# skeskinen/bert.cpp

Measured on AMD Instinct MI355X. Metric: sentences/sec (seq_len=128), higher is better.
Workload: dtype f16; 1 GPU; all-MiniLM-L6-v2 f16, batch=256 seq_len=128; per_gpu_batch=256, global_batch=256, seq_len=128, weights=f16, parallelism=dp1 (replicated weights, sharded sentences)

## Files before the change

bert.cpp_amd/csrc/device.h:

```cpp
#pragma once
#include "kernels.h"

#include <cstdio>
#include <type_traits>
#include <utility>

namespace bert_hip {

typedef _Float16 f16x2 __attribute__((ext_vector_type(2)));
typedef _Float16 f16x4 __attribute__((ext_vector_type(4)));
typedef _Float16 f16x8 __attribute__((ext_vector_type(8)));
typedef float f32x2 __attribute__((ext_vector_type(2)));
typedef float f32x4 __attribute__((ext_vector_type(4)));
typedef float f32x8 __attribute__((ext_vector_type(8)));
typedef float f32x16 __attribute__((ext_vector_type(16)));
typedef uint32_t u32x4 __attribute__((ext_vector_type(4)));
typedef uint32_t u32x16 __attribute__((ext_vector_type(16)));
typedef int32_t i32x4 __attribute__((ext_vector_type(4)));
typedef int32_t i32x16 __attribute__((ext_vector_type(16)));

template <int... I, class F>
__device__ __forceinline__ void static_for_impl(std::integer_sequence<int, I...>, F &&f) {
    (f(std::integral_constant<int, I>{}), ...);
}
// ... 52 lines not shown
}
template <bool MEMORY, int OFF, class V = f16x8>
__device__ __forceinline__ V lds_read_b128(unsigned addr) {
    static_assert(sizeof(V) == 16, "ds_read_b128 reads 16 bytes");
    static_assert(OFF >= 0 && OFF < 65536, "ds offset field is 16 bits");
    V v;
    if constexpr (MEMORY) asm volatile("ds_read_b128 %0, %1 offset:%2" : "=v"(v) : "v"(addr), "n"(OFF) : "memory");
    else asm volatile("ds_read_b128 %0, %1 offset:%2" : "=v"(v) : "v"(addr), "n"(OFF));
    return v;
}
template <class V>
__device__ __forceinline__ void landed(V &v) { asm volatile("" : "+v"(v)); }
template <int VM>
__device__ __forceinline__ void dma_barrier() {
    asm volatile("s_waitcnt vmcnt(%0) lgkmcnt(0)\n\ts_barrier" : : "n"(VM) : "memory");
}

__device__ __forceinline__ int off64(int row, int chunk) { return row * 128 + ((chunk ^ ((row >> 1) & 7)) << 4); }

__device__ __forceinline__ float rounded_f32(float v) {
    asm("" : "+v"(v));
    return v;
}

__device__ __forceinline__ void xor32_pair(float &a, float &b) {
    asm("s_nop 1\n\tv_permlane32_swap_b32 %0, %1\n\ts_nop 1" : "+v"(a), "+v"(b));
}
__device__ __forceinline__ f16x8 result_to_operand_fragment(const f16x8 &v) {
    const u32x4 d = __builtin_bit_cast(u32x4, v);
    uint32_t d0 = d[0], d1 = d[1], d2 = d[2], d3 = d[3];
    asm("s_nop 1\n\tv_permlane32_swap_b32 %0, %2\n\tv_permlane32_swap_b32 %1, %3\n\ts_nop 1" : "+v"(d0), "+v"(d1), "+v"(d2), "+v"(d3));
    return __builtin_bit_cast(f16x8, u32x4{d0, d1, d2, d3});
}
__device__ __forceinline__ float xor32_sum(float v) { float a = v, b = v; xor32_pair(a, b); return a + b; }
__device__ __forceinline__ float xor32_max(float v) { float a = v, b = v; xor32_pair(a, b); return __builtin_fmaxf(a, b); }
__device__ __forceinline__ float wave_sum_f32(float v) {
    v = xor32_sum(v);
    v += __builtin_bit_cast(float, __builtin_amdgcn_ds_swizzle(__builtin_bit_cast(int, v), (16 << 10) | 0x1F));
    v += __builtin_bit_cast(float, __builtin_amdgcn_ds_swizzle(__builtin_bit_cast(int, v), (8 << 10) | 0x1F));
    v += __builtin_bit_cast(float, __builtin_amdgcn_ds_swizzle(__builtin_bit_cast(int, v), (4 << 10) | 0x1F));
    v += __builtin_bit_cast(float, __builtin_amdgcn_mov_dpp(__builtin_bit_cast(int, v), 0x4E, 0xF, 0xF, true));
    v += __builtin_bit_cast(float, __builtin_amdgcn_mov_dpp(__builtin_bit_cast(int, v), 0xB1, 0xF, 0xF, true));
    return v;
}

#ifndef BERT_HIP_EXP16
#define BERT_HIP_EXP16 0
#endif
#if BERT_HIP_EXP16
typedef u32x4 sm_arg_t;
typedef u32x4 sm_exp_t;
__device__ __forceinline__ sm_arg_t softmax_args4(float s0, float s1, float s2, float s3, float s4, float s5, float s6, float s7, float sc, float m) {
    uint32_t a0, a1, a2, a3;
    asm("v_fma_mixlo_f16 %0, %4, %12, -%13\n\t"
        "v_fma_mixlo_f16 %1, %6, %12, -%13\n\t"
        "v_fma_mixlo_f16 %2, %8, %12, -%13\n\t"
        "v_fma_mixlo_f16 %3, %10, %12, -%13\n\t"
        "v_fma_mixhi_f16 %0, %5, %12, -%13\n\t"
        "v_fma_mixhi_f16 %1, %7, %12, -%13\n\t"
        "v_fma_mixhi_f16 %2, %9, %12, -%13\n\t"
        "v_fma_mixhi_f16 %3, %11, %12, -%13"
        : "=&v"(a0), "=&v"(a1), "=&v"(a2), "=&v"(a3)
        : "v"(s0), "v"(s1), "v"(s2), "v"(s3), "v"(s4), "v"(s5), "v"(s6), "v"(s7), "s"(sc), "v"(m));
    return u32x4{a0, a1, a2, a3};
}
__device__ __forceinline__ sm_exp_t softmax_exp4(sm_arg_t a) {
// ... 214 lines not shown
```

bert.cpp_amd/csrc/engine.hip:

```cpp
#include "engine.h"

#include <algorithm>
#include <cstdio>
#include <cstdlib>
#include <chrono>
#include <cstring>
#include <system_error>
#include <thread>

namespace bert_hip {

#define HIP_OK(expr, errvar, ret)                                                                       \
    do {                                                                                                \
        hipError_t e__ = (expr);                                                                        \
        if (e__ != hipSuccess) {                                                                        \
            errvar = std::string(#expr) + ": " + hipGetErrorString(e__);                                \
            return ret;                                                                                 \
        }                                                                                               \
    } while (0)

DevBuf::~DevBuf() {
    if (p) (void)hipFree(p);
}
bool DevBuf::alloc(size_t n, std::string &err) {
// ... 349 lines not shown
    HIP_OK(hipDeviceSynchronize(), err, -1);
    int st = 0;
    HIP_OK(hipMemcpy(&st, status_.p, sizeof(int), hipMemcpyDeviceToHost), err, -1);
    if (st) HIP_OK(hipMemset(status_.p, 0, sizeof(int)), err, -1);
    return st;
}

void Engine::set_option(const std::string &key, const std::string &value) {
#ifndef BERT_HIP_TEST_ROUTES
    if ((key == "gemm" || key == "attn") && value == "naive") {
        fprintf(stderr, "bert_hip_set_option: %s=naive is a test cross-check (libbert_test.so), not a route of libbert.so; ignored\n", key.c_str());
        return;
    }
#endif
    if (key == "gemm") {
        bool have = true;
        for (auto *L : layers_)
            for (GemmWeightStore *w : {&L->qkv, &L->o, &L->ffi, &L->ffo}) have = have && w->w.naive16 != nullptr;
        if (value == "naive" && !have)
            fprintf(stderr, "bert_hip_set_option: gemm=naive needs BERT_HIP_KERNELS=naive at load time (the f16 row-major images were not built); ignored\n");
        else gemm_naive_ = value == "naive";
    } else if (key == "attn") attn_naive_ = value == "naive";
    else if (key == "qkv2") qkv2_ = value != "0";
    else if (key == "gemm256") gemm256_ = value != "0";
    else if (key == "ln_fold" && value != "0" && !fold_images_)
        fprintf(stderr, "bert_hip_set_option: ln_fold=1 needs BERT_HIP_LN_FOLD=1 at load time (the folded images were not built); ignored\n");
    else if (key == "ln_fold") ln_fold_ = value != "0";
    else if (key == "tail") tail_ = value != "0";
    else if (key == "latency") latency_ = value != "0";
    else if (key == "stage_kernel") stage_kernel_ = value != "0";
    else if (key == "window_slots") set_window_slots(atoi(value.c_str()));
    else if (key == "latency_tokens") { const int v = atoi(value.c_str()); if (v >= 32) latency_tokens_ = v; }
    else if (key == "one_launch") one_launch_ = value == "0" ? 0 : value == "2" ? 2 : 1;
    else if (key == "f32") f32_exact_ = value != "f16";
    else if (key == "chunk_tokens") { const int v = atoi(value.c_str()); if (v > 0) chunk_tokens_ = v; }
    else if (key == "profile_replay") {
        const size_t c = value.rfind(':');
        replay_name_ = c == std::string::npos ? value : value.substr(0, c);
        replay_k_ = c == std::string::npos ? 10 : std::max(1, atoi(value.c_str() + c + 1));
    }
}

bool Engine::ensure_workspace(int t_pad, int n_sentences, std::string &err) {
    const size_t H = hp_.n_embd, I = hp_.n_intermediate, tp = (size_t)t_pad;
    const size_t es = f32_file_ ? 4 : 2;
    return x_.ensure(tp * H * es, err) && qkv_.ensure(tp * 3 * H * es, err) && ctx_.ensure(tp * H * es, err) &&
           y_.ensure(tp * H * es, err) && ff_.ensure(tp * I * es, err) && v32_.ensure((size_t)std::max(128, std::min(t_pad, (latency_tokens_ + 255) / 256 * 256)) * H * 4, err) &&
           d_out_.ensure((size_t)n_sentences * H * 4, err) &&
           windows_.ensure((size_t)n_sentences * sizeof(int2), err) &&
           (!(H > 384 && H % 256 == 0) || (ln_stats1_.ensure(tp * (2 * H / 256) * 8, err) && ln_stats2_.ensure(tp * (2 * H / 256) * 8, err) &&
                                           ln_rows1_.ensure(tp * 16, err) && ln_rows2_.ensure(tp * 16, err)));
}

template <class F>
void Engine::timed(const char *name, double flops, hipStream_t s, F &&f) {
    if (!profiling_) { f(); return; }
    auto get = [&]() {
        hipEvent_t ev;
        if (!ev_pool_.empty()) { ev = ev_pool_.back(); ev_pool_.pop_back(); }
        else (void)hipEventCreate(&ev);
        return ev;
    };
    if (!replay_name_.empty()) {
        f();
        if (replay_done_ || replay_name_ != name) return;
        replay_done_ = true;
// ... 453 lines not shown
```

bert.cpp_amd/csrc/layer_tail.hip:

```cpp
#include "device.h"

namespace bert_hip {

namespace {

constexpr int LT_TILE = 16384;
#ifndef LT_ABLATE
#define LT_ABLATE 0
#endif
#ifndef LT_UPRIO
#define LT_UPRIO 1
#endif
#ifndef LT_GELU_BATCH
#define LT_GELU_BATCH 0
#endif
#ifndef LT_DMA_SPLIT
#define LT_DMA_SPLIT 1
#endif
#ifndef LT_DPRIO
#define LT_DPRIO 0
#endif

#ifdef BERT_HIP_TIMELINE
static __device__ unsigned long long g_tl_tail[256 * 512];
// ... 25 lines not shown
    asm volatile("s_waitcnt lgkmcnt(%4)" : "+v"(f[0]), "+v"(f[1]), "+v"(f[2]), "+v"(f[3]) : "n"(N) : "memory");
}
template <int N>
__device__ __forceinline__ void wait_lgkm() {
    asm volatile("s_waitcnt lgkmcnt(%0)" : : "n"(N) : "memory");
}
template <int VM>
__device__ __forceinline__ void close_interval(f16x8 (&f)[4]) {
    asm volatile("s_waitcnt vmcnt(%4) lgkmcnt(0)\n\ts_barrier" : "+v"(f[0]), "+v"(f[1]), "+v"(f[2]), "+v"(f[3]) : "n"(VM) : "memory");
}
template <int OFF>
__device__ __forceinline__ f16x8 frag_read(unsigned addr) {
    if (LT_ABLATE & 4) { f16x8 z = (f16x8)(_Float16)0.f; asm volatile("" : "+v"(z) : "v"(addr)); return z; }
    return lds_read_b128<true, OFF>(addr);
}

__device__ __forceinline__ void dma_m0(unsigned lds) {
    if (LT_ABLATE & 1) return;
    asm volatile("s_mov_b32 m0, %0" : : "s"(lds) : "memory");
}
template <int PIECE>
__device__ __forceinline__ void dma_piece(const char *gbase, unsigned voff) {
    if (LT_ABLATE & 1) return;
    asm volatile("global_load_lds_dwordx4 %0, %1 offset:%2" : : "v"(voff), "s"(gbase - PIECE * 1024), "n"(PIECE * 1024) : "memory");
}

__device__ __forceinline__ f32x16 mfma16(const f16x8 &a, const f16x8 &b, const f32x16 &c) {
    if (LT_ABLATE & 8) { f32x16 r = c; asm volatile("" : "+v"(r[0]) : "v"(a), "v"(b)); return r; }
    return __builtin_amdgcn_mfma_f32_32x32x16_f16(a, b, c, 0, 0, 0);
}

}

template <int NT, int WT, bool RAGGED, bool HANDOVER>
__device__ __forceinline__ void layer_tail_body(const TailArgs &a, char *smem, const int tok0, const int rows, const int tid,
                                                [[maybe_unused]] f16x8 (&xnext)[8 * NT]) {
    static_assert(!(HANDOVER && RAGGED), "a ragged window's rows are packed: its lanes are not the window phase's slots");
    constexpr bool Q4 = WT != GW_F16;
    constexpr int VMQ = Q4 ? 63 : 0;
    constexpr int H = 128 * NT, NBH = 2 * NT, NB = 4 * NT, NQ = 8 * NT, NYH = 4 * NT;
    constexpr int P = NT * NT;
    constexpr int NG = NT;
    constexpr int LAGT = NT + NG;
    const int I = a.I, NC = I / 64;
    const int lane = tid & 63;
    const int wave = __builtin_amdgcn_readfirstlane(tid >> 6);
    const int t = wave & 3, role = wave >> 2;
    const int l31 = lane & 31, hi = lane >> 5;
    const int tok_w = tok0 + t * 32;
    const int row_l = RAGGED ? tok0 + min(t * 32 + l31, rows - 1) : tok_w + l31;

    char *ringU = smem;
    char *ringD = smem + 3 * LT_TILE;
    char *G = smem + 6 * LT_TILE;
    float *ST = (float *)(G + 32768);
    float *cbo = ST + 8 * 64;
    float *cg1 = cbo + H, *cbe1 = cg1 + H, *cb2 = cbe1 + H, *cg2 = cb2 + H, *cbe2 = cg2 + H, *cb1 = cbe2 + H;

    {
        constexpr int NPB = 4;
        const float *const src[6] = {a.bo, a.g1, a.be1, a.b2, a.g2, a.be2};
        float pv[6];
        f32x4 bq[NPB];
#pragma unroll
        for (int k = 0; k < 6; ++k) pv[k] = tid < H ? src[k][tid] : 0.f;
#pragma unroll
        for (int k = 0; k < NPB; ++k) {
            const int i4 = (k * 512 + tid) * 4;
            bq[k] = i4 < I ? *(const f32x4 *)(a.b1 + i4) : f32x4{0.f, 0.f, 0.f, 0.f};
        }
        if (tid < H) {
#pragma unroll
            for (int k = 0; k < 6; ++k) cbo[k * H + tid] = pv[k];
        }
#pragma unroll
        for (int k = 0; k < NPB; ++k) {
            const int i4 = (k * 512 + tid) * 4;
            if (i4 < I + 128) *(f32x4 *)(cb1 + i4) = bq[k];
        }
    }
    f32x16 accp[NBH];
    f16x4 xv[NBH][4];
    {
        const half_t *xr = a.x + (size_t)row_l * H + role * 64 + 4 * hi;
#pragma unroll
        for (int b = 0; b < NBH; ++b)
#pragma unroll
            for (int gq = 0; gq < 4; ++gq) xv[b][gq] = *(const f16x4 *)(xr + (b >> 1) * 128 + (b & 1) * 32 + 8 * gq);
    }
    f16x8 bf[NQ];
    {
        const half_t *cw = a.ctx + (size_t)row_l * H + 8 * hi;
#pragma unroll
        for (int q = 0; q < NQ; ++q) bf[q] = *(const f16x8 *)(cw + 16 * q);
    }

    auto rows_offset = [&](int pitch) __attribute__((always_inline)) {
        int ln = lane;
        asm volatile("" : "+v"(ln));
        const int ch0 = (ln & 7) ^ (ln >> 4), row = t * 32 + (ln >> 3);
        return (unsigned)(row * pitch * 2 + ch0 * 16);
    };
    const half_t *const wo = a.wo, *const w1p = a.w1p, *const w2p = a.w2p;
    auto dma128 = [&](const half_t *base, unsigned oe, int row_bytes, unsigned tile) __attribute__((always_inline)) {
        const char *b = (const char *)base;
        dma_m0(tile + (unsigned)(t * 4096));
        dma_piece<0>(b, oe);
        dma_piece<1>(b + (size_t)8 * row_bytes, oe ^ 64u);
        dma_piece<2>(b + (size_t)16 * row_bytes, oe);
        dma_piece<3>(b + (size_t)24 * row_bytes, oe ^ 64u);
    };
    const unsigned ldsU = lds_addr(ringU), ldsD = lds_addr(ringD);
    const unsigned offH = rows_offset(H);
    auto up_offset = [&]() __attribute__((always_inline)) {
        int ln = lane;
        asm volatile("" : "+v"(ln));
        return (unsigned)((t * 16 + (ln >> 4)) * H * 2 + (((ln & 15) ^ (ln >> 4)) * 16));
    };
    auto dma_up_f16 = [&](int c, int j, unsigned offU, unsigned tile) __attribute__((always_inline)) {
        const char *b = (const char *)(w1p + (size_t)c * 64 * H + j * 128);
        dma_m0(tile + (unsigned)(t * 4096));
        dma_piece<0>(b, offU);
        dma_piece<1>(b + (size_t)4 * H * 2, offU ^ 64u);
        dma_piece<2>(b + (size_t)8 * H * 2, offU ^ 128u);
// ... 43 lines not shown
    const unsigned aUp = lds_addr(ringU) + (unsigned)(l31 * 256 + ((hi ^ (l31 & 15)) << 4));

    int slot = 0;
    [[maybe_unused]] int tl = 1;
    [[maybe_unused]] const bool tlU = tid == 0, tlD = tid == 256;
    LT_STAMP(tlU, 0);
    auto pre_close = [&]() __attribute__((always_inline)) { LT_STAMP_FINE(tlU, 128 + tl); LT_STAMP_FINE(tlD, 256 + tl); };
    auto next_slot = [&]() __attribute__((always_inline)) { slot = slot == 2 ? 0 : slot + 1; LT_STAMP(tlU, tl); ++tl; };
    auto slot_plus2 = [&]() __attribute__((always_inline)) { return slot == 0 ? 2 : slot - 1; };
    [[maybe_unused]] auto slot_plus1 = [&]() __attribute__((always_inline)) { return slot == 2 ? 0 : slot + 1; };
    using PLAIN = std::false_type; using PERMUTED = std::true_type;

    auto proj_request = [&](int p, int s) __attribute__((always_inline)) {
        const int n3 = p / NT, q = p % NT;
        if (role == 0) dma_proj(n3, 2 * q, ldsU + s * LT_TILE);
        else dma_proj(n3, 2 * q + 1, ldsD + s * LT_TILE);
    };
    proj_request(0, 0);
    q4_expand_rows(PLAIN{}, role ? ringD : ringU);
    proj_request(1, 1);
    LT_STAMP(tlU, 384);
    asm volatile("s_waitcnt vmcnt(0) lgkmcnt(0)\n\ts_barrier" ::: "memory");
    LT_STAMP(tlU, 385);
#pragma unroll
    for (int b = 0; b < NBH; ++b)
#pragma unroll
        for (int gq = 0; gq < 4; ++gq) {
            const f32x4 bv = *(const f32x4 *)(cbo + (b >> 1) * 128 + role * 64 + (b & 1) * 32 + 8 * gq + 4 * hi);
#pragma unroll
            for (int e = 0; e < 4; ++e) accp[b][4 * gq + e] = (float)xv[b][gq][e] + bv[e];
        }
#pragma unroll
    for (int b = 0; b < NBH; ++b) asm volatile("" : "+v"(accp[b]));
    __builtin_amdgcn_s_waitcnt(0xc07f);
    static_for<P>([&](auto p_tag) __attribute__((always_inline)) {
        constexpr int p = decltype(p_tag)::value, n3 = p / NT, q = p % NT, p2 = p + 2;
        const unsigned bA = aR + (unsigned)(slot * LT_TILE + role * 8192), bB = bA + 3 * LT_TILE;
        f16x8 Fa[4], Fb[4];
        auto rd = [&](unsigned base, int g2, f16x8 (&F)[4]) __attribute__((always_inline)) {
            const unsigned a0 = base ^ (unsigned)((2 * g2) << 5), a1 = base ^ (unsigned)((2 * g2 + 1) << 5);
            F[0] = frag_read<0>(a0); F[1] = frag_read<4096>(a0);
            F[2] = frag_read<0>(a1); F[3] = frag_read<4096>(a1);
        };
        auto mm = [&](f16x8 (&F)[4], int ks) __attribute__((always_inline)) {
            accp[n3 * 2 + 0] = mfma16(F[0], bf[ks], accp[n3 * 2 + 0]);
            accp[n3 * 2 + 1] = mfma16(F[1], bf[ks], accp[n3 * 2 + 1]);
            accp[n3 * 2 + 0] = mfma16(F[2], bf[ks + 1], accp[n3 * 2 + 0]);
            accp[n3 * 2 + 1] = mfma16(F[3], bf[ks + 1], accp[n3 * 2 + 1]);
        };
        auto q4_turn = [&]() __attribute__((always_inline)) {
            if constexpr (p + 1 < P) q4_expand_rows(PLAIN{}, (role ? ringD : ringU) + slot_plus1() * LT_TILE);
            else if (role == 1) q4_expand_up(ringU + slot_plus1() * LT_TILE);
            const int s2 = slot_plus2();
            if constexpr (p2 < P) proj_request(p2, s2);
            else if (role == 1) dma_up(0, p2 - P, up_offset(), ldsU + s2 * LT_TILE);
        };
        constexpr int QW = Q4 && p + 1 < P ? 4 : 0;
        if constexpr (LT_ABLATE & 64) {
            if constexpr (Q4) q4_turn();
            else {
                const int s2 = slot_plus2();
                if constexpr (p2 < P) proj_request(p2, s2);
                else if (role == 1) dma_up(0, p2 - P, up_offset(), ldsU + s2 * LT_TILE);
            }
            pre_close();
            if (p2 < P || role == 1) dma_barrier<Q4 ? 63 : 4>(); else dma_barrier<VMQ>();
            next_slot();
            return;
        }
        rd(bA, 0, Fa);
        rd(bA, 1, Fb);
        if constexpr (!Q4) {
            const int s2 = slot_plus2();
            if constexpr (p2 < P) proj_request(p2, s2);
            else if (role == 1) dma_up(0, p2 - P, up_offset(), ldsU + s2 * LT_TILE);
        }
        wait_frags<4>(Fa);
        mm(Fa, 8 * q + 0);
        __builtin_amdgcn_sched_barrier(0);
        rd(bB, 0, Fa);
        wait_frags<4>(Fb);
        mm(Fb, 8 * q + 2);
        __builtin_amdgcn_sched_barrier(0);
        rd(bB, 1, Fb);
        if constexpr (Q4) { q4_turn(); __builtin_amdgcn_sched_barrier(0); }
        wait_frags<4 + QW>(Fa);
        mm(Fa, 8 * q + 4);
        __builtin_amdgcn_sched_barrier(0);
        wait_frags<0>(Fb);
        mm(Fb, 8 * q + 6);
        __builtin_amdgcn_sched_barrier(0);
        pre_close();
        if (p2 < P || role == 1) dma_barrier<Q4 ? 63 : 4>(); else dma_barrier<VMQ>();
        next_slot();
    });

    if (role == 1) q4_expand_up(ringU + slot_plus1() * LT_TILE);
    LT_STAMP(tlU, 386); LT_STAMP(tlD, 396);
    float ln_rstd, ln_nmr;
    {
        float s1 = 0.f, s2 = 0.f;
#pragma unroll
        for (int b = 0; b < ((LT_ABLATE & 32) ? 0 : NBH); ++b)
#pragma unroll
            for (int r = 0; r < 16; ++r) { s1 += accp[b][r]; s2 = __builtin_fmaf(accp[b][r], accp[b][r], s2); }
        s1 += __shfl_xor(s1, 32);
        s2 += __shfl_xor(s2, 32);
        if (hi == 0) *(f32x2 *)(ST + wave * 64 + l31 * 2) = f32x2{s1, s2};
        LT_STAMP(tlU, 387); LT_STAMP(tlD, 397);
        asm volatile("s_waitcnt lgkmcnt(0)\n\ts_barrier" ::: "memory");
        LT_STAMP(tlU, 388);
        const f32x2 o = *(const f32x2 *)(ST + (wave ^ 4) * 64 + l31 * 2);
        s1 += o[0]; s2 += o[1];
        layernorm_scale(s1, s2, 1.0f / H, ln_rstd, ln_nmr);
    }
    auto normalise_block = [&](auto b_tag, f16x8 &y0, f16x8 &y1) __attribute__((always_inline)) {
        constexpr int b = decltype(b_tag)::value;
        const int f0 = (b >> 1) * 128 + role * 64 + (b & 1) * 32 + 4 * hi;
        if constexpr (LT_ABLATE & 32) {
#pragma unroll
            for (int e = 0; e < 8; ++e) { y0[e] = (_Float16)accp[b][e]; y1[e] = (_Float16)accp[b][8 + e]; }
            return;
// ... 466 lines not shown
```

bert.cpp_amd/csrc/model_kernel.hip:

```cpp
#define BERT_HIP_PHASES_ONLY
#include "qkv_attention2.hip"
#include "layer_tail.hip"
#undef BERT_HIP_PHASES_ONLY
#include "pool_normalize.h"

namespace bert_hip {

#ifdef BERT_HIP_MODEL_TIMELINE
static __device__ unsigned long long g_tl_model[1024 * 32];
#define MK_STAMP(i) do { const int mk_i = (i); if (threadIdx.x == 0 && mk_i < 32) g_tl_model[(blockIdx.x & 1023) * 32 + mk_i] = __builtin_amdgcn_s_memrealtime(); } while (0)
#else
#define MK_STAMP(i) do { } while (0)
#endif

namespace {

constexpr int MODEL_MAX_LAYERS = 12;

struct ModelLayerArgs {
    const half_t *wqkv, *wo, *w1p, *w2p;
    const float *bqkv, *bo, *g1, *be1, *b1, *b2, *g2, *be2;
};
struct ModelArgs {
    half_t *x, *ctx;
    const int32_t *cu;
    const int2 *groups;
    const int *n_groups;
    int n_layer, n_head, n_sent, I, slot_mask;
    float *pooled;
    int *status;
    int max_len;
    ModelLayerArgs layer[MODEL_MAX_LAYERS];
};

}

template <int NT, bool RAGGED>
__global__ __launch_bounds__(512, 2) void model_kernel(ModelArgs m) {
    extern __shared__ __attribute__((aligned(16))) char smem[];
    const int window = (int)blockIdx.x;
    int tok0 = window * 128, rows = 128, first = window, count = 1;
    if constexpr (RAGGED) {
        if (m.groups) {
            if (m.n_groups && window >= *m.n_groups) return;
            const int2 g = m.groups[window];
            first = g.x; count = g.y;
        }
        if (count <= 0 || first >= m.n_sent) return;
        tok0 = m.cu[first];
        rows = min(m.cu[first + count] - tok0, 128);
    }
    const int wave_index = __builtin_amdgcn_readfirstlane((int)threadIdx.x >> 6);
    auto thread_id = [&]() __attribute__((always_inline)) {
        int ln = (int)__builtin_amdgcn_mbcnt_hi(~0u, __builtin_amdgcn_mbcnt_lo(~0u, 0u)), w = wave_index;
        asm volatile("" : "+v"(ln), "+s"(w));
        return w * 64 + ln;
    };
    MK_STAMP(0);
    const int n_layer = rows > 0 ? m.n_layer : 0;
    auto window_phase = [&](const ModelLayerArgs &L, auto xregs_tag, const f16x8 *xf) __attribute__((always_inline)) {
        const int tid = thread_id();
        Qkv2Args q;
        q.x = m.x; q.w = L.wqkv; q.qs = nullptr; q.sc = nullptr; q.bias = L.bqkv; q.cu = m.cu; q.groups = RAGGED ? m.groups : nullptr; q.n_groups = nullptr;
        q.out = m.ctx; q.n_head = m.n_head; q.n_sent = m.n_sent; q.spw = 1; q.slot_mask = m.slot_mask;
        qkv_attention2_body<2 * NT, NT, GW_F16, !RAGGED, decltype(xregs_tag)::value>(q, smem, window, tid, xf);
    };
    auto tail_phase = [&](const ModelLayerArgs &L, f16x8 (&xf)[8 * NT]) __attribute__((always_inline)) {
        const int tid = thread_id();
        TailArgs t;
        t.ctx = m.ctx; t.x = m.x; t.wo = L.wo; t.w1p = L.w1p; t.w2p = L.w2p;
        t.wo_qs = t.w1_qs = t.w2_qs = nullptr; t.wo_sc = t.w1_sc = t.w2_sc = nullptr;
        t.bo = L.bo; t.g1 = L.g1; t.be1 = L.be1; t.b1 = L.b1; t.b2 = L.b2; t.g2 = L.g2; t.be2 = L.be2; t.out = m.x; t.I = m.I;
        layer_tail_body<NT, GW_F16, RAGGED, !RAGGED>(t, smem, tok0, rows, tid, xf);
    };
    auto hand_over = [&]() __attribute__((always_inline)) {
        __builtin_amdgcn_fence(__ATOMIC_RELEASE, "workgroup");
        asm volatile("s_waitcnt vmcnt(0) lgkmcnt(0)\n\ts_barrier" ::: "memory");
        __builtin_amdgcn_fence(__ATOMIC_ACQUIRE, "workgroup");
    };
    if constexpr (RAGGED) {
        for (int l = 0; l < n_layer; ++l) {
            f16x8 none[8 * NT];
            window_phase(m.layer[l], std::false_type{}, nullptr);
            hand_over();
            MK_STAMP(1 + 2 * l);
            tail_phase(m.layer[l], none);
            hand_over();
            MK_STAMP(2 + 2 * l);
        }
    } else {
        if (n_layer > 0) window_phase(m.layer[0], std::false_type{}, nullptr);
        for (int l = 0; l < n_layer; ++l) {
            hand_over();
            MK_STAMP(1 + 2 * l);
            f16x8 xf[8 * NT];
            tail_phase(m.layer[l], xf);
            hand_over();
            MK_STAMP(2 + 2 * l);
            if (l + 1 < n_layer) window_phase(m.layer[l + 1], std::true_type{}, xf);
        }
    }
    if (m.pooled) {
        const int tid = thread_id();
        for (int j = 0; j < count; ++j) {
            const int b = first + j, t0 = m.cu[b];
            int n = m.cu[b + 1] - t0;
            if (!RAGGED && (t0 != tok0 || n != 128)) n = -1;
            pool_normalize_sentence(m.x, t0, n, b, 128 * NT, m.max_len, m.status, m.pooled, (float *)smem, tid, tid < 256);
            __syncthreads();
        }
    }
    MK_STAMP(1 + 2 * n_layer);
}

bool model_kernel_supported(const GemmWeight &Wqkv, const GemmWeight &Wo, const GemmWeight &W1, const GemmWeight &W2, int n_layer,
                            int n_head, int d_head, int max_len) {
    const int H = n_head * d_head;
    return n_layer <= MODEL_MAX_LAYERS && (H == 256 || H == 384) && max_len >= 1 && max_len <= 128 &&
           Wqkv.type == GW_F16 && Wo.type == GW_F16 && qkv_attention2_supported(Wqkv, n_head, d_head, max_len) && layer_tail_supported(Wo, W1, W2);
}

void launch_model_kernel(const ModelLayerWeights *layers, int n_layer, half_t *x, half_t *ctx, const int32_t *cu_seqlens, int n_sentences,
                         int n_tokens, const int2 *groups, int n_groups, const int *n_groups_dev, int n_head, float *pooled, int max_len,
                         int *status, int slots, hipStream_t stream) {
    ModelArgs m;
    m.pooled = pooled; m.status = status; m.max_len = max_len;
    m.x = x; m.ctx = ctx; m.cu = cu_seqlens; m.groups = groups; m.n_groups = n_groups_dev;
    m.n_layer = n_layer; m.n_head = n_head; m.n_sent = n_sentences; m.I = layers[0].W1->N; m.slot_mask = slots - 1;
    for (int l = 0; l < n_layer; ++l) {
        const ModelLayerWeights &s = layers[l];
        ModelLayerArgs &d = m.layer[l];
        d.wqkv = s.Wqkv->w16; d.wo = s.Wo->w16; d.w1p = s.W1->w16p; d.w2p = s.W2->w16p;
        d.bqkv = s.bqkv; d.bo = s.bo; d.g1 = s.g1; d.be1 = s.be1; d.b1 = s.b1; d.b2 = s.b2; d.g2 = s.g2; d.be2 = s.be2;
    }
    const int H = layers[0].W1->K, KT = H / 64, GB = KT / 2;
    const size_t lds_q = (size_t)3 * GB * Q2_TILE + 2 * (2 * Q2_WIN * 64 + 32 * Q2_VT_LD * 2) + (size_t)2 * H * sizeof(float);
    const size_t lds = std::max(lds_q, layer_tail_lds(H, m.I));
    const bool full = (long long)n_sentences * 128 == n_tokens;
    const int grid = full || !groups ? n_sentences : n_groups;
    static DeviceFlags configured[4];
    auto go = [&](auto kernel, int which) {
        configure_once(configured[which], [&] { (void)hipFuncSetAttribute((const void *)kernel, hipFuncAttributeMaxDynamicSharedMemorySize, 160 * 1024); });
        BERT_LAUNCH(kernel, dim3(grid), dim3(512), lds, stream, m);
#ifdef BERT_HIP_MODEL_TIMELINE
        static int shots = 0;
        if (grid >= 256 && shots++ == 30) {
            (void)hipDeviceSynchronize();
            static unsigned long long h[1024 * 32];
            (void)hipMemcpyFromSymbol(h, HIP_SYMBOL(g_tl_model), sizeof(h));
            const int nw = grid < 1024 ? grid : 1024, ns = 2 + 2 * n_layer;
            unsigned long long t0 = ~0ull;
            for (int w = 0; w < nw; ++w) t0 = h[w * 32] < t0 ? h[w * 32] : t0;
            fprintf(stderr, "model_kernel timeline, %d workgroups (us after the first workgroup's start: min mean max):\n", nw);
            for (int i = 0; i < ns; ++i) {
                double lo = 1e30, hi = 0, sum = 0;
                for (int w = 0; w < nw; ++w) { const double v = (double)(h[w * 32 + i] - t0) * 0.01; lo = v < lo ? v : lo; hi = v > hi ? v : hi; sum += v; }
                fprintf(stderr, "  stamp %2d: %8.2f %8.2f %8.2f\n", i, lo, sum / nw, hi);
            }
            fprintf(stderr, "  mean phase durations (window, tail) per layer:");
            for (int l = 0; l < n_layer; ++l) {
                double a = 0, b = 0;
                for (int w = 0; w < nw; ++w) { a += (double)(h[w * 32 + 1 + 2 * l] - h[w * 32 + 2 * l]) * 0.01; b += (double)(h[w * 32 + 2 + 2 * l] - h[w * 32 + 1 + 2 * l]) * 0.01; }
                fprintf(stderr, " (%.1f, %.1f)", a / nw, b / nw);
            }
            fprintf(stderr, "\n  mean end per XCD:");
            for (int x = 0; x < 8; ++x) {
                double e = 0; int c = 0;
                for (int w = x; w < nw; w += 8) { e += (double)(h[w * 32 + ns - 1] - t0) * 0.01; ++c; }
                fprintf(stderr, " %.1f", e / c);
            }
            fprintf(stderr, "\n  mean end per eighth of the grid:");
// ... 17 lines not shown
```

bert.cpp_amd/csrc/qkv_attention2.hip:

```cpp
#include "device.h"

#ifndef Q2_PM
#define Q2_PM 3
#endif
#ifndef Q2_PRIO
#define Q2_PRIO 0
#endif

namespace bert_hip {

namespace {

constexpr int Q2_WIN = 128;
constexpr int Q2_TILE = 12288;
constexpr int Q2_VT_LD = Q2_WIN + 4;

struct Qkv2Args {
    const half_t *x;
    const half_t *w;
    const uint4 *qs;
    const void *sc;
    const float *bias;
    const int32_t *cu;
    const int2 *groups;
    const int *n_groups;
    half_t *out;
    int n_head, n_sent, spw;
    int slot_mask;
};

__device__ __forceinline__ int q2_off32(int row, int chunk) { return row * 64 + ((chunk ^ ((row >> 2) & 3)) << 4); }

__device__ __forceinline__ void q2_wait6(f16x8 (&f)[2][3]) {
    asm volatile("s_waitcnt lgkmcnt(6)"
                 : "+v"(f[0][0]), "+v"(f[0][1]), "+v"(f[0][2]), "+v"(f[1][0]), "+v"(f[1][1]), "+v"(f[1][2]) : : "memory");
}
template <int VM>
__device__ __forceinline__ void q2_slab_barrier(f16x8 (&f)[2][3]) {
    asm volatile("s_waitcnt vmcnt(%6) lgkmcnt(0)\n\ts_barrier"
                 : "+v"(f[0][0]), "+v"(f[0][1]), "+v"(f[0][2]), "+v"(f[1][0]), "+v"(f[1][1]), "+v"(f[1][2]) : "n"(VM) : "memory");
}
__device__ __forceinline__ void q2_wait14(f16x8 (&f)[2][3]) {
    asm volatile("s_waitcnt lgkmcnt(14)"
                 : "+v"(f[0][0]), "+v"(f[0][1]), "+v"(f[0][2]), "+v"(f[1][0]), "+v"(f[1][1]), "+v"(f[1][2]) : : "memory");
}
__device__ __forceinline__ void q2_wait0_bias(f16x8 (&f)[2][3], f32x4 (&bq)[4], f32x4 (&bk)[4]) {
    asm volatile("s_waitcnt lgkmcnt(0)"
                 : "+v"(f[0][0]), "+v"(f[0][1]), "+v"(f[0][2]), "+v"(f[1][0]), "+v"(f[1][1]), "+v"(f[1][2]),
                   "+v"(bq[0]), "+v"(bq[1]), "+v"(bq[2]), "+v"(bq[3]), "+v"(bk[0]), "+v"(bk[1]), "+v"(bk[2]), "+v"(bk[3]) : : "memory");
}

}

template <int KT, int GB, int WT, bool FULL = false, bool XREGS = false>
__device__ __forceinline__ void qkv_attention2_body(const Qkv2Args &a, char *smem, const int window, const int tid,
                                                    [[maybe_unused]] const f16x8 *xf = nullptr) {
    static_assert(FULL || !XREGS, "fragments handed over in registers: full windows only");
    constexpr bool Q4 = WT != GW_F16;
    constexpr int H = 64 * KT, NBAR = KT / GB, SLAB = GB * Q2_TILE, PPS = 3 * GB;
    static_assert(KT == 2 * GB && NBAR == 2, "");
    constexpr int QKV_BYTES = 2 * Q2_WIN * 64 + 32 * Q2_VT_LD * 2;
    char *RING = smem;
    char *QKV = smem + 3 * SLAB;
    float *BS = (float *)(QKV + 2 * QKV_BYTES);

    const int lane = tid & 63;
    const int wave = __builtin_amdgcn_readfirstlane(tid >> 6);
    const int l31 = lane & 31, hi = lane >> 5;
    const int blk = wave & 3;
    const int n_head = a.n_head;
    TL_STAMP_AT(tid == 256, 120);
    TL_REALTIME_AT(tid == 256, 121);
    TL_STAMP_AT(tid == 0, 250);
    TL_REALTIME_AT(tid == 0, 251);

    const int wp = blk;
    const unsigned loff = (unsigned)(((wp * 8 + (lane >> 3)) * H + (((lane & 7) ^ (((wp & 1) << 2) | ((lane >> 4) & 3))) * 8)) * 2);
    auto dma_piece = [&](const char *hbase, auto j_tag, int dslot, auto i_tag) __attribute__((always_inline)) {
        constexpr int i = decltype(i_tag)::value, j = decltype(j_tag)::value, t = i / 3, rb = i % 3;
        const char *src = hbase + ((size_t)rb * H * H + (size_t)(j * GB + t) * 64) * 2;
        __builtin_amdgcn_global_load_lds(AS_GLOBAL(src + loff), AS_LDS(RING + dslot * SLAB + t * Q2_TILE + rb * 4096 + wp * 1024), 16, 0, 0);
    };
    const char *const wbase = (const char *)a.w;
    if constexpr (!Q4) {
        if (wave >= 4) static_for<PPS>([&](auto i) __attribute__((always_inline)) { dma_piece(wbase, std::integral_constant<int, 0>{}, 0, i); });
    }

    int first, count;
    if constexpr (FULL) { first = window; count = 1; }
    else {
        if (a.groups) {
            if (a.n_groups && window >= *a.n_groups) {
                asm volatile("s_waitcnt vmcnt(0)" ::: "memory");
                return;
            }
            const int2 g = a.groups[window];
            first = g.x; count = g.y;
        }
        else { first = window * a.spw; count = min(a.spw, a.n_sent - first); }
        if (count <= 0) {
            asm volatile("s_waitcnt vmcnt(0)" ::: "memory");
            return;
        }
// ... 163 lines not shown
                        pieces(hh_tag, m_tag);
                    });
                } else {
                    q2_wait0_bias(F[par], bq, bk);
                    static_for<2>([&](auto i) __attribute__((always_inline)) { mma(PAR{}, i, std::integral_constant<int, 0>{}, std::integral_constant<int, 2 * hh + decltype(i)::value>{}); });
                    pieces(hh_tag, std::integral_constant<int, 1>{});
                    static_for<2>([&](auto i) __attribute__((always_inline)) { mma(PAR{}, i, std::integral_constant<int, 1>{}, std::integral_constant<int, 2 * hh + decltype(i)::value>{}); });
#pragma unroll
                    for (int gg = 0; gg < 4; ++gg) {
                        f16x4 oq;
#pragma unroll
                        for (int e = 0; e < 4; ++e) oq[e] = (_Float16)(acc[0][4 * gg + e] + bq[gg][e]);
                        *(f16x4 *)(QS + q2_off32(slot, gg) + hi * 8) = oq;
                    }
                    static_for<2>([&](auto i) __attribute__((always_inline)) { mma(PAR{}, i, std::integral_constant<int, 2>{}, std::integral_constant<int, 2 * hh + decltype(i)::value>{}); });
                    pieces(hh_tag, std::integral_constant<int, 4>{});
#pragma unroll
                    for (int gg = 0; gg < 4; ++gg) {
                        f16x4 ok;
#pragma unroll
                        for (int e = 0; e < 4; ++e) ok[e] = (_Float16)(acc[1][4 * gg + e] + bk[gg][e]);
                        *(f16x4 *)(KS + q2_off32(slot, gg) + hi * 8) = ok;
                    }
#pragma unroll
                    for (int gg = 0; gg < 4; ++gg) {
                        f16x4 ov;
#pragma unroll
                        for (int e = 0; e < 4; ++e) ov[e] = (_Float16)(acc[2][4 * gg + e] + bv);
                        *(f16x4 *)(VT + l31 * Q2_VT_LD + blk * 32 + 8 * gg + 4 * hi) = ov;
                    }
                }
            });
            if (h < 8) TL_STAMP_AT(tl_sel, 2 + 6 * h + 4);
            dma_barrier<Q4 ? 63 : PPS>();
            if (h < 8) TL_STAMP_AT(tl_sel, 2 + 6 * h + 5);
            rslot = rslot == 2 ? 0 : rslot + 1;
            set_slot();
            read_half(std::integral_constant<int, 0>{}, std::integral_constant<int, 0>{}, std::integral_constant<int, 0>{});
        }
        TL_STAMP_AT(tl_sel, 60);
        asm volatile("s_waitcnt vmcnt(0)" ::: "memory");
    } else {
        unsigned need = 0, inner = 0;
#pragma unroll
        for (int kt = 0; kt < 4; ++kt) {
            const bool nd = gtok >= 0 && k0 < 32 * kt + 32 && k1 > 32 * kt;
            const bool in = gtok < 0 || (k0 <= 32 * kt && k1 >= 32 * kt + 32);
            if (__any(nd)) need |= 1u << kt;
            if (__all(in)) inner |= 1u << kt;
        }
        need = __builtin_amdgcn_readfirstlane(need);
        inner = __builtin_amdgcn_readfirstlane(inner);
        const unsigned klen = (unsigned)(k1 - k0);
        const int kbase = 4 * hi - k0;
        const float sc = 1.44269504088896340736f / __builtin_sqrtf(32.0f);
        for (int i = tid; i < 2 * H; i += 256) BS[i] = a.bias[i];
        asm volatile("s_waitcnt vmcnt(0) lgkmcnt(0)\n\ts_barrier" ::: "memory");

        if constexpr (Q2_PRIO > 0) __builtin_amdgcn_s_setprio(Q2_PRIO);
        [[maybe_unused]] const bool tl_sel = tid == 0;
        auto attend = [&](int hh, auto wb_tag, auto fast_tag, int tb) __attribute__((always_inline)) {
            constexpr bool WB = decltype(wb_tag)::value, FAST = decltype(fast_tag)::value;
            const char *QS = QKV + (hh & 1) * QKV_BYTES, *KS = QS + Q2_WIN * 64;
            const half_t *VT = (const half_t *)(KS + Q2_WIN * 64);
            f32x16 s[4];
            f16x8 qf[2];
#pragma unroll
            for (int kk = 0; kk < 2; ++kk) qf[kk] = *(const f16x8 *)(QS + q2_off32(slot, kk * 2 + hi));
            float mx = -INFINITY;
            int kb = kbase;
            unsigned kl = klen;
            if constexpr (!FAST) asm volatile("" : "+v"(kb), "+v"(kl));
#pragma unroll
            for (int kt = 0; kt < 4; ++kt) {
                if (FAST || (need & (1u << kt))) {
#pragma unroll
                    for (int r = 0; r < 16; ++r) s[kt][r] = 0.f;
#pragma unroll
                    for (int kk = 0; kk < 2; ++kk) {
                        const f16x8 kf = *(const f16x8 *)(KS + q2_off32(kt * 32 + l31, kk * 2 + hi));
                        s[kt] = __builtin_amdgcn_mfma_f32_32x32x16_f16(kf, qf[kk], s[kt], 0, 0, 0);
                    }
                    if (FAST || (inner & (1u << kt))) {
#pragma unroll
                        for (int r = 0; r < 16; ++r) mx = fmaxf(mx, s[kt][r]);
                    } else {
#pragma unroll
                        for (int r = 0; r < 16; ++r) {
                            const bool ok = (unsigned)(kt * 32 + (r & 3) + 8 * (r >> 2) + kb) < kl;
                            const float v = ok ? s[kt][r] : -INFINITY;
                            s[kt][r] = v;
                            mx = fmaxf(mx, v);
                        }
                    }
                }
// ... 6 lines not shown
                }
            }
            mx = xor32_max(mx) * sc;
            mx = fmaxf(mx, -3.0e38f);
            float psum = 0.f;
            f32x16 o;
#pragma unroll
            for (int r = 0; r < 16; ++r) o[r] = 0.f;
#pragma unroll
            for (int kt = 0; kt < 4; ++kt) {
                if (FAST || (need & (1u << kt))) {
#pragma unroll
                    for (int st = 0; st < 2; ++st) {
                        const f16x8 pf = softmax_p8(s[kt][8 * st], s[kt][8 * st + 1], s[kt][8 * st + 2], s[kt][8 * st + 3], s[kt][8 * st + 4],
                                                    s[kt][8 * st + 5], s[kt][8 * st + 6], s[kt][8 * st + 7], sc, mx, psum);
                        const int key0 = kt * 32 + 16 * st + 4 * hi;
                        const half_t *vr = VT + l31 * Q2_VT_LD + key0;
                        const f16x4 v0 = *(const f16x4 *)vr, v1 = *(const f16x4 *)(vr + 8);
                        f16x8 vf;
#pragma unroll
                        for (int e = 0; e < 4; ++e) { vf[e] = v0[e]; vf[4 + e] = v1[e]; }
                        o = __builtin_amdgcn_mfma_f32_32x32x16_f16(vf, pf, o, 0, 0, 0);
                    }
                }
                if constexpr (WB) {
                    if (kt + 4 == Q2_PM) {
                        if (tb < 8) TL_STAMP_AT(tl_sel, 128 + 6 * tb + 1);
                        asm volatile("s_barrier" ::: "memory");
                        if (tb < 8) TL_STAMP_AT(tl_sel, 128 + 6 * tb + 2);
                    }
                }
            }
            psum = xor32_sum(psum);
            if (gtok >= 0) {
                const float inv = 1.0f / psum;
                half_t *op = a.out + (size_t)gtok * H + hh * 32;
#pragma unroll
                for (int gq = 0; gq < 4; ++gq) {
                    f16x4 ov;
#pragma unroll
                    for (int e = 0; e < 4; ++e) ov[e] = (_Float16)rounded_f32(o[4 * gq + e] * inv);
                    *(f16x4 *)(op + 8 * gq + 4 * hi) = ov;
                }
            }
        };
        const bool fast = FULL || (need == 0xFu && inner == 0xFu);
        asm volatile("s_barrier" ::: "memory");
        asm volatile("s_barrier" ::: "memory");
        for (int h = 1; h < n_head; ++h) {
            if (h < 8) TL_STAMP_AT(tl_sel, 128 + 6 * h);
            if (FULL || fast) attend(h - 1, std::true_type{}, std::true_type{}, h);
            else if constexpr (!FULL) attend(h - 1, std::true_type{}, std::false_type{}, h);
            if (h < 8) TL_STAMP_AT(tl_sel, 128 + 6 * h + 5);
            asm volatile("s_barrier" ::: "memory");
        }
        TL_STAMP_AT(tl_sel, 190);
        if (FULL || fast) attend(n_head - 1, std::false_type{}, std::true_type{}, 0);
        else if constexpr (!FULL) attend(n_head - 1, std::false_type{}, std::false_type{}, 0);
        TL_STAMP_AT(tl_sel, 192);
        TL_STAMP_AT(tl_sel, 252);
        TL_REALTIME_AT(tl_sel, 253);
    }
}

template <int KT, int GB, int WT>
__global__ __launch_bounds__(512, 2) void qkv_attention2_kernel(Qkv2Args a) {
    extern __shared__ __attribute__((aligned(16))) char smem[];
    qkv_attention2_body<KT, GB, WT>(a, smem, (int)blockIdx.x, (int)threadIdx.x);
}

#ifndef BERT_HIP_PHASES_ONLY
constexpr int BW_THREADS = 512;

template <int SLOT>
__global__ __launch_bounds__(BW_THREADS) void build_windows_kernel(const int32_t *__restrict__ cu, int B, int2 *__restrict__ windows,
                                                                   int *__restrict__ n_windows) {
    constexpr int BW_STATES = 128 / SLOT + 1;
    __shared__ unsigned char exit_state[BW_THREADS][BW_STATES];
    __shared__ int closes[BW_THREADS][BW_STATES];
    __shared__ int opened[BW_THREADS][BW_STATES];
    __shared__ int entry_fill[BW_THREADS], entry_first[BW_THREADS], entry_index[BW_THREADS];
    const int t = threadIdx.x, per = (B + BW_THREADS - 1) / BW_THREADS, n_blocks = per ? (B + per - 1) / per : 0;
    const int b0 = min(B, t * per), b1 = min(B, b0 + per);

    int fill[BW_STATES], n_closed[BW_STATES], first[BW_STATES];
#pragma unroll
    for (int e = 0; e < BW_STATES; ++e) { fill[e] = e * SLOT; n_closed[e] = 0; first[e] = -1; }
    for (int b = b0; b < b1; ++b) {
        const int n = cu[b + 1] - cu[b];
#pragma unroll
        for (int e = 0; e < BW_STATES; ++e) {
// ... 89 lines not shown
```

Before: 336,700 sentences/s.

## Hand attention context to layer tail through registers and LDS instead of global memory

In the fused model kernel's full-window path, the attention waves now keep each head's normalized context output in registers. They exchange it through LDS so the wave layout matches what the layer tail expects, and the tail reads these fragments directly instead of writing ctx to global memory and reading it back. The last heads go through an edge area of LDS, and part of that read is deferred into the tail's GEMM pipeline. This removes a global round trip per layer, at the cost of higher register pressure, extra barriers and tight LDS-map constraints. A test-only option that poisons ctx is also added to check that the global buffer is no longer read.

```diff
diff --git a/bert.cpp_amd/csrc/device.h b/bert.cpp_amd/csrc/device.h
--- a/bert.cpp_amd/csrc/device.h
+++ b/bert.cpp_amd/csrc/device.h
@@ -108,6 +108,7 @@
     asm("s_nop 1\n\tv_permlane32_swap_b32 %0, %2\n\tv_permlane32_swap_b32 %1, %3\n\ts_nop 1" : "+v"(d0), "+v"(d1), "+v"(d2), "+v"(d3));
     return __builtin_bit_cast(f16x8, u32x4{d0, d1, d2, d3});
 }
+constexpr int ctx_edge_offset(int nq) { return nq * 4096 > 80 * 1024 ? nq * 4096 : 80 * 1024; }
 __device__ __forceinline__ float xor32_sum(float v) { float a = v, b = v; xor32_pair(a, b); return a + b; }
 __device__ __forceinline__ float xor32_max(float v) { float a = v, b = v; xor32_pair(a, b); return __builtin_fmaxf(a, b); }
 __device__ __forceinline__ float wave_sum_f32(float v) {
diff --git a/bert.cpp_amd/csrc/engine.hip b/bert.cpp_amd/csrc/engine.hip
--- a/bert.cpp_amd/csrc/engine.hip
+++ b/bert.cpp_amd/csrc/engine.hip
@@ -405,6 +405,14 @@
     else if (key == "window_slots") set_window_slots(atoi(value.c_str()));
     else if (key == "latency_tokens") { const int v = atoi(value.c_str()); if (v >= 32) latency_tokens_ = v; }
     else if (key == "one_launch") one_launch_ = value == "0" ? 0 : value == "2" ? 2 : 1;
+#ifdef BERT_HIP_TEST_ROUTES
+    else if (key == "test_poison_ctx") {
+        (void)hipSetDevice(device());
+        (void)hipDeviceSynchronize();
+        if (ctx_.p) (void)hipMemset(ctx_.p, 0xFF, ctx_.bytes);
+        (void)hipDeviceSynchronize();
+    }
+#endif
     else if (key == "f32") f32_exact_ = value != "f16";
     else if (key == "chunk_tokens") { const int v = atoi(value.c_str()); if (v > 0) chunk_tokens_ = v; }
     else if (key == "profile_replay") {
diff --git a/bert.cpp_amd/csrc/layer_tail.hip b/bert.cpp_amd/csrc/layer_tail.hip
--- a/bert.cpp_amd/csrc/layer_tail.hip
+++ b/bert.cpp_amd/csrc/layer_tail.hip
@@ -81,10 +81,11 @@
 
 }
 
-template <int NT, int WT, bool RAGGED, bool HANDOVER>
+template <int NT, int WT, bool RAGGED, bool HANDOVER, bool CTXREGS = false>
 __device__ __forceinline__ void layer_tail_body(const TailArgs &a, char *smem, const int tok0, const int rows, const int tid,
-                                                [[maybe_unused]] f16x8 (&xnext)[8 * NT]) {
+                                                [[maybe_unused]] f16x8 (&xnext)[8 * NT], [[maybe_unused]] const f16x8 *cf = nullptr) {
     static_assert(!(HANDOVER && RAGGED), "a ragged window's rows are packed: its lanes are not the window phase's slots");
+    static_assert(!(CTXREGS && RAGGED), "a ragged window's rows are packed: its lanes are not the attention waves' queries");
     constexpr bool Q4 = WT != GW_F16;
     constexpr int VMQ = Q4 ? 63 : 0;
     constexpr int H = 128 * NT, NBH = 2 * NT, NB = 4 * NT, NQ = 8 * NT, NYH = 4 * NT;
@@ -138,7 +139,16 @@
             for (int gq = 0; gq < 4; ++gq) xv[b][gq] = *(const f16x4 *)(xr + (b >> 1) * 128 + (b & 1) * 32 + 8 * gq);
     }
     f16x8 bf[NQ];
-    {
+    constexpr bool CTX_LATE = CTXREGS && ctx_edge_offset(NQ) >= 6 * LT_TILE && ctx_edge_offset(NQ) + 16384 <= 6 * LT_TILE + 32768;
+    if constexpr (CTXREGS) {
+        static_assert(ctx_edge_offset(NQ) >= 5 * LT_TILE && ctx_edge_offset(NQ) + 16384 <= 6 * LT_TILE + 32768,
+                      "the edge area: ringD's third slot or G, where the prologue's DMA and parameter writes do not reach");
+#pragma unroll
+        for (int q = 0; q < NQ - 4; ++q) bf[q] = cf[q];
+        const char *const er = smem + ctx_edge_offset(NQ) + t * 4096 + lane * 16;
+#pragma unroll
+        for (int q = 0; q < (CTX_LATE ? 0 : 4); ++q) bf[NQ - 4 + q] = *(const f16x8 *)(er + q * 1024);
+    } else {
         const half_t *cw = a.ctx + (size_t)row_l * H + 8 * hi;
 #pragma unroll
         for (int q = 0; q < NQ; ++q) bf[q] = *(const f16x8 *)(cw + 16 * q);
@@ -248,6 +258,11 @@
         }
 #pragma unroll
     for (int b = 0; b < NBH; ++b) asm volatile("" : "+v"(accp[b]));
+    if constexpr (CTXREGS) {
+#pragma unroll
+        for (int q = 0; q < (CTX_LATE ? NQ - 4 : NQ); ++q) asm volatile("" : "+v"(bf[q]));
+    }
+    [[maybe_unused]] const unsigned aEdge = CTX_LATE ? lds_addr(smem) + (unsigned)(ctx_edge_offset(NQ) + t * 4096 + lane * 16) : 0u;
     __builtin_amdgcn_s_waitcnt(0xc07f);
     static_for<P>([&](auto p_tag) __attribute__((always_inline)) {
         constexpr int p = decltype(p_tag)::value, n3 = p / NT, q = p % NT, p2 = p + 2;
@@ -294,16 +309,26 @@
         wait_frags<4>(Fa);
         mm(Fa, 8 * q + 0);
         __builtin_amdgcn_sched_barrier(0);
+        if constexpr (CTX_LATE && q == NT - 1) {
+            bf[NQ - 4] = lds_read_b128<true, 0>(aEdge);
+            bf[NQ - 3] = lds_read_b128<true, 1024>(aEdge);
+        }
         rd(bB, 0, Fa);
         wait_frags<4>(Fb);
+        if constexpr (CTX_LATE && q == NT - 1) { landed(bf[NQ - 4]); landed(bf[NQ - 3]); }
         mm(Fb, 8 * q + 2);
         __builtin_amdgcn_sched_barrier(0);
+        if constexpr (CTX_LATE && q == NT - 1) {
+            bf[NQ - 2] = lds_read_b128<true, 2048>(aEdge);
+            bf[NQ - 1] = lds_read_b128<true, 3072>(aEdge);
+        }
         rd(bB, 1, Fb);
         if constexpr (Q4) { q4_turn(); __builtin_amdgcn_sched_barrier(0); }
         wait_frags<4 + QW>(Fa);
         mm(Fa, 8 * q + 4);
         __builtin_amdgcn_sched_barrier(0);
         wait_frags<0>(Fb);
+        if constexpr (CTX_LATE && q == NT - 1) { landed(bf[NQ - 2]); landed(bf[NQ - 1]); }
         mm(Fb, 8 * q + 6);
         __builtin_amdgcn_sched_barrier(0);
         pre_close();
diff --git a/bert.cpp_amd/csrc/model_kernel.hip b/bert.cpp_amd/csrc/model_kernel.hip
--- a/bert.cpp_amd/csrc/model_kernel.hip
+++ b/bert.cpp_amd/csrc/model_kernel.hip
@@ -3,6 +3,8 @@
 #include "layer_tail.hip"
 #undef BERT_HIP_PHASES_ONLY
 #include "pool_normalize.h"
+
+#include <cstdlib>
 
 namespace bert_hip {
 
@@ -58,20 +60,20 @@
     };
     MK_STAMP(0);
     const int n_layer = rows > 0 ? m.n_layer : 0;
-    auto window_phase = [&](const ModelLayerArgs &L, auto xregs_tag, const f16x8 *xf) __attribute__((always_inline)) {
+    auto window_phase = [&](const ModelLayerArgs &L, auto xregs_tag, const f16x8 *xf, f16x8 *cf) __attribute__((always_inline)) {
         const int tid = thread_id();
         Qkv2Args q;
         q.x = m.x; q.w = L.wqkv; q.qs = nullptr; q.sc = nullptr; q.bias = L.bqkv; q.cu = m.cu; q.groups = RAGGED ? m.groups : nullptr; q.n_groups = nullptr;
         q.out = m.ctx; q.n_head = m.n_head; q.n_sent = m.n_sent; q.spw = 1; q.slot_mask = m.slot_mask;
-        qkv_attention2_body<2 * NT, NT, GW_F16, !RAGGED, decltype(xregs_tag)::value>(q, smem, window, tid, xf);
+        qkv_attention2_body<2 * NT, NT, GW_F16, !RAGGED, decltype(xregs_tag)::value, !RAGGED>(q, smem, window, tid, xf, cf);
     };
-    auto tail_phase = [&](const ModelLayerArgs &L, f16x8 (&xf)[8 * NT]) __attribute__((always_inline)) {
+    auto tail_phase = [&](const ModelLayerArgs &L, f16x8 (&xf)[8 * NT], const f16x8 *cf) __attribute__((always_inline)) {
         const int tid = thread_id();
         TailArgs t;
         t.ctx = m.ctx; t.x = m.x; t.wo = L.wo; t.w1p = L.w1p; t.w2p = L.w2p;
         t.wo_qs = t.w1_qs = t.w2_qs = nullptr; t.wo_sc = t.w1_sc = t.w2_sc = nullptr;
         t.bo = L.bo; t.g1 = L.g1; t.be1 = L.be1; t.b1 = L.b1; t.b2 = L.b2; t.g2 = L.g2; t.be2 = L.be2; t.out = m.x; t.I = m.I;
-        layer_tail_body<NT, GW_F16, RAGGED, !RAGGED>(t, smem, tok0, rows, tid, xf);
+        layer_tail_body<NT, GW_F16, RAGGED, !RAGGED, !RAGGED>(t, smem, tok0, rows, tid, xf, cf);
     };
     auto hand_over = [&]() __attribute__((always_inline)) {
         __builtin_amdgcn_fence(__ATOMIC_RELEASE, "workgroup");
@@ -81,23 +83,28 @@
     if constexpr (RAGGED) {
         for (int l = 0; l < n_layer; ++l) {
             f16x8 none[8 * NT];
-            window_phase(m.layer[l], std::false_type{}, nullptr);
+            window_phase(m.layer[l], std::false_type{}, nullptr, nullptr);
             hand_over();
             MK_STAMP(1 + 2 * l);
-            tail_phase(m.layer[l], none);
+            tail_phase(m.layer[l], none, nullptr);
             hand_over();
             MK_STAMP(2 + 2 * l);
         }
     } else {
-        if (n_layer > 0) window_phase(m.layer[0], std::false_type{}, nullptr);
+        f16x8 cf[8 * NT];
+        if (n_layer > 0) window_phase(m.layer[0], std::false_type{}, nullptr, cf);
         for (int l = 0; l < n_layer; ++l) {
             hand_over();
             MK_STAMP(1 + 2 * l);
             f16x8 xf[8 * NT];
-            tail_phase(m.layer[l], xf);
+            tail_phase(m.layer[l], xf, cf);
             hand_over();
             MK_STAMP(2 + 2 * l);
-            if (l + 1 < n_layer) window_phase(m.layer[l + 1], std::true_type{}, xf);
+            if (l + 1 < n_layer) window_phase(m.layer[l + 1], std::true_type{}, xf, cf);
+            else {
+#pragma unroll
+                for (int q = 0; q < 8 * NT; ++q) asm volatile("" : "=v"(cf[q]));
+            }
         }
     }
     if (m.pooled) {
@@ -137,6 +144,7 @@
     const size_t lds_q = (size_t)3 * GB * Q2_TILE + 2 * (2 * Q2_WIN * 64 + 32 * Q2_VT_LD * 2) + (size_t)2 * H * sizeof(float);
     const size_t lds = std::max(lds_q, layer_tail_lds(H, m.I));
     const bool full = (long long)n_sentences * 128 == n_tokens;
+    if (n_head * 32 != H) { fprintf(stderr, "launch_model_kernel: n_head %d x 32 != H %d\n", n_head, H); abort(); }
     const int grid = full || !groups ? n_sentences : n_groups;
     static DeviceFlags configured[4];
     auto go = [&](auto kernel, int which) {
diff --git a/bert.cpp_amd/csrc/qkv_attention2.hip b/bert.cpp_amd/csrc/qkv_attention2.hip
--- a/bert.cpp_amd/csrc/qkv_attention2.hip
+++ b/bert.cpp_amd/csrc/qkv_attention2.hip
@@ -52,10 +52,13 @@
 
 }
 
-template <int KT, int GB, int WT, bool FULL = false, bool XREGS = false>
+template <int KT, int GB, int WT, bool FULL = false, bool XREGS = false, bool CTXREGS = false>
 __device__ __forceinline__ void qkv_attention2_body(const Qkv2Args &a, char *smem, const int window, const int tid,
-                                                    [[maybe_unused]] const f16x8 *xf = nullptr) {
+                                                    [[maybe_unused]] const f16x8 *xf = nullptr,
+                                                    [[maybe_unused]] f16x8 *cf = nullptr) {
     static_assert(FULL || !XREGS, "fragments handed over in registers: full windows only");
+    static_assert(!CTXREGS || (FULL && WT == GW_F16), "the context in registers: full windows, f16 weights");
+    constexpr int NCF = 4 * KT;
     constexpr bool Q4 = WT != GW_F16;
     constexpr int H = 64 * KT, NBAR = KT / GB, SLAB = GB * Q2_TILE, PPS = 3 * GB;
     static_assert(KT == 2 * GB && NBAR == 2, "");
@@ -69,6 +72,10 @@
     const int l31 = lane & 31, hi = lane >> 5;
     const int blk = wave & 3;
     const int n_head = a.n_head;
+    if constexpr (CTXREGS) {
+        static_assert(NCF * 4096 <= 3 * SLAB && ctx_edge_offset(NCF) >= NCF * 4096 && ctx_edge_offset(NCF) + 16384 <= 3 * SLAB + QKV_BYTES &&
+                      ((2 * KT - 1) & 1) == 1, "the context exchange does not fit the window phase's LDS map");
+    }
     TL_STAMP_AT(tid == 256, 120);
     TL_REALTIME_AT(tid == 256, 121);
     TL_STAMP_AT(tid == 0, 250);
@@ -298,14 +305,32 @@
                 }
             });
             if (h < 8) TL_STAMP_AT(tl_sel, 2 + 6 * h + 4);
+            if constexpr (CTXREGS) {
+                if (h + 1 == n_head) dma_barrier<0>(); else dma_barrier<PPS>();
+            } else
             dma_barrier<Q4 ? 63 : PPS>();
             if (h < 8) TL_STAMP_AT(tl_sel, 2 + 6 * h + 5);
+            if constexpr (CTXREGS) {
+                if (h + 1 < n_head) {
+                    rslot = rslot == 2 ? 0 : rslot + 1;
+                    set_slot();
+                    read_half(std::integral_constant<int, 0>{}, std::integral_constant<int, 0>{}, std::integral_constant<int, 0>{});
+                }
+            } else {
             rslot = rslot == 2 ? 0 : rslot + 1;
             set_slot();
             read_half(std::integral_constant<int, 0>{}, std::integral_constant<int, 0>{}, std::integral_constant<int, 0>{});
+            }
         }
         TL_STAMP_AT(tl_sel, 60);
-        asm volatile("s_waitcnt vmcnt(0)" ::: "memory");
+        if constexpr (!CTXREGS) asm volatile("s_waitcnt vmcnt(0)" ::: "memory");
+        if constexpr (CTXREGS) {
+            asm volatile("s_waitcnt lgkmcnt(0)\n\ts_barrier" ::: "memory");
+            const char *const xr = smem + blk * (NCF * 1024) + lane * 16;
+#pragma unroll
+            for (int q = 0; q < NCF - 4; ++q) cf[q] = *(const f16x8 *)(xr + q * 1024);
+            __builtin_amdgcn_s_waitcnt(0xc07f);
+        }
     } else {
         unsigned need = 0, inner = 0;
 #pragma unroll
@@ -325,8 +350,14 @@
 
         if constexpr (Q2_PRIO > 0) __builtin_amdgcn_s_setprio(Q2_PRIO);
         [[maybe_unused]] const bool tl_sel = tid == 0;
-        auto attend = [&](int hh, auto wb_tag, auto fast_tag, int tb) __attribute__((always_inline)) {
+        if constexpr (CTXREGS) {
+#pragma unroll
+            for (int q = 0; q < NCF - 4; ++q) asm volatile("" : "=v"(cf[q]));
+        }
+        [[maybe_unused]] f16x8 pen0, pen1;
+        auto attend = [&](int hh, auto wb_tag, auto fast_tag, int tb, [[maybe_unused]] auto to_tag) __attribute__((always_inline)) {
             constexpr bool WB = decltype(wb_tag)::value, FAST = decltype(fast_tag)::value;
+            [[maybe_unused]] constexpr int TO = decltype(to_tag)::value;
             const char *QS = QKV + (hh & 1) * QKV_BYTES, *KS = QS + Q2_WIN * 64;
             const half_t *VT = (const half_t *)(KS + Q2_WIN * 64);
             f32x16 s[4];
@@ -399,6 +430,28 @@
                 }
             }
             psum = xor32_sum(psum);
+            if constexpr (CTXREGS) {
+                const float inv = 1.0f / psum;
+                f16x8 r0, r1;
+#pragma unroll
+                for (int e = 0; e < 8; ++e) { r0[e] = (_Float16)rounded_f32(o[e] * inv); r1[e] = (_Float16)rounded_f32(o[8 + e] * inv); }
+                r0 = result_to_operand_fragment(r0);
+                r1 = result_to_operand_fragment(r1);
+                if constexpr (TO == 0)
+                    static_for<2 * KT - 2>([&](auto i_tag) __attribute__((always_inline)) {
+                        constexpr int i = decltype(i_tag)::value;
+                        if (hh == i) {
+                            cf[2 * i] = r0; cf[2 * i + 1] = r1;
+                            asm volatile("" : "+v"(cf[2 * i]), "+v"(cf[2 * i + 1]));
+                        }
+                    });
+                else if constexpr (TO == 1) { pen0 = r0; pen1 = r1; }
+                else {
+                    char *const ew = smem + ctx_edge_offset(NCF) + blk * 4096 + lane * 16;
+                    *(f16x8 *)(ew + 2048) = r0;
+                    *(f16x8 *)(ew + 3072) = r1;
+                }
+            } else
             if (gtok >= 0) {
                 const float inv = 1.0f / psum;
                 half_t *op = a.out + (size_t)gtok * H + hh * 32;
@@ -414,16 +467,33 @@
         const bool fast = FULL || (need == 0xFu && inner == 0xFu);
         asm volatile("s_barrier" ::: "memory");
         asm volatile("s_barrier" ::: "memory");
-        for (int h = 1; h < n_head; ++h) {
+        using TO0 = std::integral_constant<int, 0>;
+        for (int h = 1; h < (CTXREGS ? n_head - 1 : n_head); ++h) {
             if (h < 8) TL_STAMP_AT(tl_sel, 128 + 6 * h);
-            if (FULL || fast) attend(h - 1, std::true_type{}, std::true_type{}, h);
-            else if constexpr (!FULL) attend(h - 1, std::true_type{}, std::false_type{}, h);
+            if (FULL || fast) attend(h - 1, std::true_type{}, std::true_type{}, h, TO0{});
+            else if constexpr (!FULL) attend(h - 1, std::true_type{}, std::false_type{}, h, TO0{});
             if (h < 8) TL_STAMP_AT(tl_sel, 128 + 6 * h + 5);
             asm volatile("s_barrier" ::: "memory");
         }
+        if constexpr (CTXREGS) {
+            if (n_head - 1 < 8) TL_STAMP_AT(tl_sel, 128 + 6 * (n_head - 1));
+            attend(n_head - 2, std::true_type{}, std::true_type{}, n_head - 1, std::integral_constant<int, 1>{});
+            if (n_head - 1 < 8) TL_STAMP_AT(tl_sel, 128 + 6 * (n_head - 1) + 5);
+            asm volatile("s_barrier" ::: "memory");
+        }
         TL_STAMP_AT(tl_sel, 190);
-        if (FULL || fast) attend(n_head - 1, std::false_type{}, std::true_type{}, 0);
-        else if constexpr (!FULL) attend(n_head - 1, std::false_type{}, std::false_type{}, 0);
+        if constexpr (CTXREGS) {
+            char *const xw = smem + blk * (NCF * 1024) + lane * 16;
+#pragma unroll
+            for (int q = 0; q < NCF - 4; ++q) *(f16x8 *)(xw + q * 1024) = cf[q];
+            char *const ew = smem + ctx_edge_offset(NCF) + blk * 4096 + lane * 16;
+            *(f16x8 *)ew = pen0;
+            *(f16x8 *)(ew + 1024) = pen1;
+            asm volatile("s_waitcnt lgkmcnt(0)\n\ts_barrier" ::: "memory");
+        }
+        if constexpr (CTXREGS) attend(n_head - 1, std::false_type{}, std::true_type{}, 0, std::integral_constant<int, 2>{});
+        else if (FULL || fast) attend(n_head - 1, std::false_type{}, std::true_type{}, 0, TO0{});
+        else if constexpr (!FULL) attend(n_head - 1, std::false_type{}, std::false_type{}, 0, TO0{});
         TL_STAMP_AT(tl_sel, 192);
         TL_STAMP_AT(tl_sel, 252);
         TL_REALTIME_AT(tl_sel, 253);
```

New measurement: 348,500 sentences/s (median of 6 runs). 1.03x the previous value.
